# mika314/melonix

Measured on AMD Instinct MI355X. Metric: STFT+pitch+resynth frames/sec (48 kHz, 4096 FFT, 256 hop); % HBM roofline, higher is better.
Workload: dtype f32

## Files before the change

### melonix_amd/csrc/stft_core.h

```cpp
#pragma once
#include <stdint.h>
#include <type_traits>

#if defined(__HIPCC__)
#include <hip/hip_runtime.h>
#define MX_HD __host__ __device__ __forceinline__
namespace mx {
using cpx = float2;
}
#else
#define MX_HD inline __attribute__((always_inline))
namespace mx {
struct alignas(8) cpx {
  float x, y;
};
}
#endif

namespace mx {

#include "stft_consts.inc"

MX_HD cpx mk(float x, float y) {
  cpx r;
  r.x = x;
  r.y = y;
  return r;
}
MX_HD float fma_(float a, float b, float c) { return __builtin_fmaf(a, b, c); }
MX_HD cpx cadd(cpx a, cpx b) { return mk(a.x + b.x, a.y + b.y); }
MX_HD cpx csub(cpx a, cpx b) { return mk(a.x - b.x, a.y - b.y); }
MX_HD cpx cmul(cpx a, cpx b) { return mk(fma_(a.x, b.x, -(a.y * b.y)), fma_(a.x, b.y, a.y * b.x)); }
MX_HD float cnorm2(cpx a) { return fma_(a.x, a.x, a.y * a.y); }
MX_HD cpx cconj(cpx a) { return mk(a.x, -a.y); }
MX_HD cpx csel(bool c, cpx a, cpx b) { return mk(c ? a.x : b.x, c ? a.y : b.y); }
MX_HD float fast_sqrt(float x) {
#if defined(__HIP_DEVICE_COMPILE__)
  return __builtin_amdgcn_sqrtf(x);
#else
  return __builtin_sqrtf(x);
#endif
}
MX_HD constexpr int ilog2(int x) { return x <= 1 ? 0 : 1 + ilog2(x >> 1); }

}
#include "pk_math.h"
namespace mx {

template <int K>
MX_HD cpx mulw64(cpx a) {
  constexpr int k = ((K % 64) + 64) % 64;
  constexpr float h = 0.707106781187f;
  if constexpr (k == 0) return a;
  else if constexpr (k == 16) return mk(a.y, -a.x);
  else if constexpr (k == 32) return mk(-a.x, -a.y);
  else if constexpr (k == 48) return mk(-a.y, a.x);
  else if constexpr (k == 8) return mk(h * (a.x + a.y), h * (a.y - a.x));
  else if constexpr (k == 24) return mk(h * (a.y - a.x), -h * (a.x + a.y));
  else if constexpr (k == 40) return mk(-h * (a.x + a.y), h * (a.x - a.y));
  else if constexpr (k == 56) return mk(h * (a.x - a.y), h * (a.x + a.y));
  else {
    constexpr float c = kCos64[k], s = kSin64[k];
    return mk(fma_(a.x, c, a.y * s), fma_(a.y, c, -(a.x * s)));
  }
}

template <int K>
MX_HD void bfly_w64(cpx E, cpx O, cpx &out0, cpx &out1) {
  constexpr int k = ((K % 64) + 64) % 64;
  if constexpr (k == 0) {
    pk_bfly_1(E, O, out0, out1);
  } else if constexpr (k == 16) {
    pk_bfly_mi(E, O, out0, out1);
  } else if constexpr (k == 32) {
    pk_bfly_1(E, O, out1, out0);
  } else if constexpr (k == 48) {
    pk_bfly_mi(E, O, out1, out0);
  } else {
    pk_bfly_cs(E, O, mk(kCos64[k], kSin64[k]), out0, out1);
  }
}

template <int R, int Q>
struct Combine {
  static MX_HD void run(const cpx *E, const cpx *O, cpx *out) {
    bfly_w64<Q * 64 / R>(E[Q], O[Q], out[Q], out[Q + R / 2]);
    if constexpr (Q + 1 < R / 2) Combine<R, Q + 1>::run(E, O, out);
  }
};

template <int R>
struct Dft {
  static MX_HD void run(const cpx *in, cpx *out) {
    cpx e[R / 2], o[R / 2], E[R / 2], O[R / 2];
#pragma unroll
    for (int q = 0; q < R / 2; ++q) {
      e[q] = in[2 * q];
      o[q] = in[2 * q + 1];
    }
    Dft<R / 2>::run(e, E);
    Dft<R / 2>::run(o, O);
    Combine<R, 0>::run(E, O, out);
  }
};
template <>
struct Dft<2> {
  static MX_HD void run(const cpx *in, cpx *out) {
    pk_bfly_1(in[0], in[1], out[0], out[1]);
  }
};
template <>
struct Dft<1> {
  static MX_HD void run(const cpx *in, cpx *out) { out[0] = in[0]; }
};

template <int R, int S, int O0, bool CONJ>
struct DftTw {
  static MX_HD void run(const cpx *v, const cpx *w, cpx *out) {
    if constexpr (R == 2) {
      constexpr int i0 = O0, i1 = O0 + S;
      if constexpr (i0 == 0) pk_leaf0_tw<CONJ>(v[0], v[i1], w[i1], out[0], out[1]);
      else pk_leaf_tw<CONJ>(v[i0], w[i0], v[i1], w[i1], out[0], out[1]);
    } else {
      cpx E[R / 2], O[R / 2];
      DftTw<R / 2, 2 * S, O0, CONJ>::run(v, w, E);
      DftTw<R / 2, 2 * S, O0 + S, CONJ>::run(v, w, O);
      Combine<R, 0>::run(E, O, out);
    }
  }
};

template <int N_, int E_>
struct Plan {
  static constexpr int N = N_;
  static constexpr int M = N / 2;
  static constexpr int E = E_;
  static constexpr int T = M / E;
  static constexpr int R3 = E / 2;
  static constexpr int R1 = (N == 4096) ? 16 : 32;
  static constexpr int R2 = M / (R1 * R3);
  static constexpr int NS3 = R1 * R2;
  static constexpr int NB1 = E / R1;
  static constexpr int NB2 = E / R2;
  static constexpr int TW2 = (R2 - 1) * R1;
  static constexpr int TW3 = (R3 - 1) * NS3;
  static constexpr int L1 = ilog2(R1);
  static_assert(N == 4096 || N == 16384 || N == 32768, "supported FFT sizes");
  static_assert((N == 4096) ? E == 16 : E == 32, "supported points per thread");
  static_assert(R1 * R2 * R3 == M && R2 <= E && R1 <= E && T % 64 == 0, "radix plan must cover M");
};

template <class P>
MX_HD constexpr bool t1_padded() { return P::R1 == 32; }
template <class P>
MX_HD constexpr int t1_size() { return t1_padded<P>() ? P::M + P::M / 32 : P::M; }
template <class P>
MX_HD int t1_index(int i) {
  if constexpr (t1_padded<P>()) return i + (i >> 5);
  else return i ^ ((i >> P::L1) & 15);
}

struct alignas(4) f2u {
  float x, y;
};
template <bool ALIGNED8>
MX_HD cpx ld_pair(const float *base, int i) {
  const char *a = reinterpret_cast<const char *>(base) + (size_t)(4u * (unsigned)i);
  if constexpr (ALIGNED8) {
    return *reinterpret_cast<const cpx *>(a);
  } else {
    const f2u u = *reinterpret_cast<const f2u *>(a);
    return mk(u.x, u.y);
  }
}

MX_HD float ld_one(const float *base, int i) {
  return *reinterpret_cast<const float *>(reinterpret_cast<const char *>(base) + (size_t)(4u * (unsigned)i));
}

template <class P, int WSTEP, bool ALIGNED8>
MX_HD void load_frame(int t, cpx (&Y)[P::E], const float *x, const float *w) {
#pragma unroll
  for (int e = 0; e < P::E; ++e) {
    const int p = 2 * (t + P::T * e);
    cpx xs, ws;
    if constexpr (ALIGNED8 && WSTEP == 1) {
      xs = ld_pair<true>(x, p);
      ws = ld_pair<true>(w, p);
    } else {
      xs = ld_pair<false>(x, p);
      if constexpr (WSTEP == 1) {
        ws = ld_pair<false>(w, p);
      } else {
        const f2u wu = *reinterpret_cast<const f2u *>(w - p - 1);
        ws = mk(wu.y, wu.x);
      }
    }
    Y[e] = pk_mul(xs, ws);
  }
}

template <int T>
MX_HD constexpr float win_grow(int e) {
  return T == 64 ? kWinGrow64[e] : T == 128 ? kWinGrow128[e] : T == 256 ? kWinGrow256[e] : kWinGrow512[e];
}
template <class P, bool CLAMP = true>
MX_HD cpx geo_weight(cpx a0, int e) {
  constexpr float sc = 0.5f / (float)P::N;
  const float g = e == 0 ? 1.0f : win_grow<P::T>(e);
  const cpx w = e == 0 ? a0 : mk(a0.x * g, a0.y * g);
  if constexpr (!CLAMP) {
    return w;
  } else {
    const unsigned sb = __builtin_bit_cast(unsigned, sc), xb = __builtin_bit_cast(unsigned, w.x), yb = __builtin_bit_cast(unsigned, w.y);
    return mk(__builtin_bit_cast(float, xb < sb ? xb : sb), __builtin_bit_cast(float, yb < sb ? yb : sb));
  }
}
template <class P>
MX_HD int geo_clamped_slots(int hop) { return (hop + 2 * P::T - 1) / (2 * P::T); }
constexpr int kGeoTail = 2;
template <class P, bool ALIGNED8>
MX_HD void load_frame_geo(int t, cpx (&Y)[P::E], const float *x, const float *wb, int hop) {
  static_assert(P::T == 64 || P::T == 128 || P::T == 256 || P::T == 512, "growth table per T");
  static_assert(P::E <= 32, "growth table length");
  const cpx a0 = ld_pair<true>(wb, 2 * t);
  if (geo_clamped_slots<P>(hop) <= kGeoTail) {
#pragma unroll
    for (int e = 0; e < P::E; ++e) {
      const cpx xs = ld_pair<ALIGNED8>(x, 2 * (t + P::T * e));
      Y[e] = pk_mul(xs, e < P::E - kGeoTail ? geo_weight<P, false>(a0, e) : geo_weight<P, true>(a0, e));
    }
  } else {
#pragma unroll
    for (int e = 0; e < P::E; ++e) Y[e] = pk_mul(ld_pair<ALIGNED8>(x, 2 * (t + P::T * e)), geo_weight<P, true>(a0, e));
  }
}

template <class P>
MX_HD void apply_window_geo(int t, cpx (&Y)[P::E], const cpx (&xr)[P::E], const float *wb, int hop) {
  const cpx a0 = ld_pair<true>(wb, 2 * t);
  if (geo_clamped_slots<P>(hop) <= kGeoTail) {
#pragma unroll
    for (int e = 0; e < P::E; ++e)
      Y[e] = pk_mul(xr[e], e < P::E - kGeoTail ? geo_weight<P, false>(a0, e) : geo_weight<P, true>(a0, e));
  } else {
#pragma unroll
    for (int e = 0; e < P::E; ++e) Y[e] = pk_mul(xr[e], geo_weight<P, true>(a0, e));
  }
}

template <class P, bool ALIGNED8>
MX_HD void load_raw(int t, cpx (&xr)[P::E], const float *x) {
#pragma unroll
  for (int e = 0; e < P::E; ++e) {
    xr[e] = ld_pair<ALIGNED8>(x, 2 * (t + P::T * e));
  }
}
template <class P, int WSTEP, bool ALIGNED8>
MX_HD void apply_window(int t, cpx (&Y)[P::E], const cpx (&xr)[P::E], const float *w) {
#pragma unroll
  for (int e = 0; e < P::E; ++e) {
    const int p = 2 * (t + P::T * e);
    cpx ws;
    if constexpr (WSTEP == 1) {
      ws = ld_pair<ALIGNED8>(w, p);
    } else {
      const f2u wu = *reinterpret_cast<const f2u *>(w - p - 1);
      ws = mk(wu.y, wu.x);
    }
    Y[e] = pk_mul(xr[e], ws);
  }
}

template <class P>
MX_HD void pass1(const cpx (&Y)[P::E], cpx (&v)[P::E]) {
#pragma unroll
  for (int b = 0; b < P::NB1; ++b) {
    cpx in[P::R1], out[P::R1];
#pragma unroll
    for (int r = 0; r < P::R1; ++r) in[r] = Y[b + P::NB1 * r];
    Dft<P::R1>::run(in, out);
#pragma unroll
    for (int r = 0; r < P::R1; ++r) v[b * P::R1 + r] = out[r];
  }
}

template <class P, int HOP>
struct Slide {
  static constexpr int H = HOP / 2;
  static constexpr bool ok = (HOP > 0) && (HOP % 2 == 0) && (H % P::T == 0) && (2 * (H / P::T) <= P::E);
  static constexpr int D = ok ? H / P::T : 1;
};

template <class P, int HOP>
MX_HD void slide_edge(int t, const float *wtab, float inv_sc, cpx (&edge)[Slide<P, HOP>::D]) {
  using S = Slide<P, HOP>;
#pragma unroll
  for (int i = 0; i < S::D; ++i) {
    const int p = 2 * (t + P::T * (P::E - 2 * S::D + i));
    edge[i] = mk(wtab[p] * inv_sc, wtab[p + 1] * inv_sc);
  }
}

template <class P, int HOP>
MX_HD void slide_fetch(int t, const float *xe, cpx (&nx)[Slide<P, HOP>::D]) {
  using S = Slide<P, HOP>;
#pragma unroll
  for (int i = 0; i < S::D; ++i) nx[i] = *reinterpret_cast<const cpx *>(xe - HOP + 2 * (t + P::T * i));
}

template <class P, int HOP>
MX_HD void slide_step(cpx (&Y)[P::E], const cpx (&nx)[Slide<P, HOP>::D], const cpx (&edge)[Slide<P, HOP>::D],
                      float g, float sc) {
  using S = Slide<P, HOP>;
  const cpx gg = mk(g, g), ss = mk(sc, sc);
#pragma unroll
  for (int e = 0; e < P::E - 2 * S::D; ++e) Y[e] = pk_mul_xs(Y[e + S::D], gg);
#pragma unroll
  for (int i = 0; i < S::D; ++i) Y[P::E - 2 * S::D + i] = pk_mul(Y[P::E - S::D + i], edge[i]);
#pragma unroll
  for (int i = 0; i < S::D; ++i) Y[P::E - S::D + i] = pk_mul_xs(nx[i], ss);
}


template <class P>
struct Circ {
  static constexpr int W = 2 * P::T;
  static constexpr int CS = (P::T == 128) ? 4 : (P::T == 256) ? 3 : 2;
  static MX_HD bool ok(int hop) { return hop >= 1 && hop <= (CS - 1) * P::T && hop <= 2 * W; }
  static constexpr int slot(int k) { return (P::E - (CS - 1) + k) & (P::E - 1); }
};
template <class P>
struct CircGeo {
  int o;
  int s;
  int cr;
  int len;
};
template <class P>
MX_HD CircGeo<P> circ_geo(long long frame_end, int hop) {
  constexpr int W = Circ<P>::W;
  const long long start = frame_end - P::N;
  CircGeo<P> g;
  g.o = (int)(start & (long long)(W - 1));
  g.s = ((int)((start - hop) & (long long)(W - 1)) + hop) / W;
  g.len = 2 * hop;
  g.cr = (g.o - g.len) & (P::N - 1);
  return g;
}
template <class P>
MX_HD void circ_load_first(int t, cpx (&Y)[P::E], const float *xa, const float *w, int o) {
#pragma unroll
  for (int e = 0; e < P::E; ++e) {
    const int c2 = 2 * (t + P::T * e);
    const int q0 = (c2 - o) & (P::N - 1), q1 = (c2 + 1 - o) & (P::N - 1);
    Y[e] = mk(xa[q0] * w[q0], xa[q1] * w[q1]);
  }
}
template <class P>
MX_HD void circ_fetch(int t, const float *xs, const float *wt, const CircGeo<P> &g, float (&px)[2 * Circ<P>::CS],
                      float (&pw)[2 * Circ<P>::CS]) {
#pragma unroll
  for (int k = 0; k < Circ<P>::CS; ++k) {
    const int c2 = 2 * (t + P::T * Circ<P>::slot(k));
    int d0 = (c2 - g.cr) & (P::N - 1), d1 = (c2 + 1 - g.cr) & (P::N - 1);
    d0 = d0 < g.len ? d0 : g.len - 1;
    d1 = d1 < g.len ? d1 : g.len - 1;
    px[2 * k] = ld_one(xs, d0);
    px[2 * k + 1] = ld_one(xs, d1);
    pw[2 * k] = ld_one(wt, d0);
    pw[2 * k + 1] = ld_one(wt, d1);
  }
}
template <class P, int S>
MX_HD void circ_age(cpx (&Y)[P::E], cpx gg) {
  cpx head[S > 0 ? S : 1];
#pragma unroll
  for (int i = 0; i < S; ++i) head[i] = Y[i];
#pragma unroll
  for (int e = 0; e < P::E - S; ++e) Y[e] = pk_mul_xs(Y[e + S], gg);
#pragma unroll
  for (int i = 0; i < S; ++i) Y[P::E - S + i] = pk_mul_xs(head[i], gg);
}
template <class P>
MX_HD void circ_step(int t, cpx (&Y)[P::E], float decay, const CircGeo<P> &g, const float (&px)[2 * Circ<P>::CS],
                     const float (&pw)[2 * Circ<P>::CS]) {
  const cpx gg = mk(decay, decay);
  constexpr int SMAX = (Circ<P>::W - 1 + (Circ<P>::CS - 1) * P::T) / Circ<P>::W;
  static_assert(SMAX <= 2, "rotations by 0, 1 or 2 slots");
  if (g.s == 0) circ_age<P, 0>(Y, gg);
  else if (SMAX == 1 || g.s == 1) circ_age<P, 1>(Y, gg);
  else circ_age<P, 2>(Y, gg);
#pragma unroll
  for (int k = 0; k < Circ<P>::CS; ++k) {
    const int e = Circ<P>::slot(k);
    const int c2 = 2 * (t + P::T * e);
    const int d0 = (c2 - g.cr) & (P::N - 1), d1 = (c2 + 1 - g.cr) & (P::N - 1);
    const float n0 = px[2 * k] * pw[2 * k], n1 = px[2 * k + 1] * pw[2 * k + 1];
    Y[e] = mk(d0 < g.len ? n0 : Y[e].x, d1 < g.len ? n1 : Y[e].y);
  }
}


#if defined(__HIP_DEVICE_COMPILE__)
#define MX_LDS_ASM 1
typedef float mx_f2v __attribute__((ext_vector_type(2)));
template <int OFF>
__device__ __forceinline__ mx_f2v lds_rd64(uint32_t addr) {
  static_assert(OFF >= 0 && OFF < 163840, "LDS is 160 KiB");
  mx_f2v r;
  if constexpr (OFF < 65536) {
    asm volatile("ds_read_b64 %0, %1 offset:%2" : "=v"(r) : "v"(addr), "n"(OFF) : "memory");
  } else {
    const uint32_t hi = addr + (uint32_t)(OFF & ~65535);
    asm volatile("ds_read_b64 %0, %1 offset:%2" : "=v"(r) : "v"(hi), "n"(OFF & 65535) : "memory");
  }
  return r;
}
__device__ __forceinline__ uint32_t lds_addr(const void *p) {
  return (uint32_t)(uintptr_t)(const __attribute__((address_space(3))) void *)p;
}
template <int N>
__device__ __forceinline__ void lds_wait(mx_f2v (&q)[N]) {
  static_assert(N % 8 == 0, "tied in groups of 8");
  asm volatile("s_waitcnt lgkmcnt(0)" ::: "memory");
#pragma unroll
  for (int i = 0; i < N; i += 8)
    asm volatile("" : "+v"(q[i]), "+v"(q[i + 1]), "+v"(q[i + 2]), "+v"(q[i + 3]), "+v"(q[i + 4]),
                 "+v"(q[i + 5]), "+v"(q[i + 6]), "+v"(q[i + 7]));
}
#endif
template <int I, int N, class F>
MX_HD void static_for(F &&f) {
  if constexpr (I < N) {
    f(std::integral_constant<int, I>{});
    static_for<I + 1, N>(f);
  }
}

template <class P>
MX_HD void store_t1(int t, const cpx (&v)[P::E], cpx *lds) {
  if constexpr (t1_padded<P>()) {
    static_assert(P::R1 <= 32 && (P::T * P::R1) % 32 == 0, "T1 padding is one point per 32");
    cpx *const p = lds + (t * P::R1 + ((t * P::R1) >> 5));
#pragma unroll
    for (int b = 0; b < P::NB1; ++b) {
#pragma unroll
      for (int r = 0; r < P::R1; ++r) p[b * (P::T * P::R1 + P::T * P::R1 / 32) + r] = v[b * P::R1 + r];
    }
  } else {
    const unsigned B8 = (unsigned)((t * P::R1) ^ (t & 15)) << 3;
    char *const base = reinterpret_cast<char *>(lds);
#pragma unroll
    for (int r = 0; r < P::R1; ++r) {
      cpx *p = reinterpret_cast<cpx *>(base + (B8 ^ ((unsigned)r << 3)));
#pragma unroll
      for (int b = 0; b < P::NB1; ++b) p[b * P::T * P::R1] = v[b * P::R1 + r];
    }
  }
}

template <class P>
struct T1Read {
  static constexpr int S = P::M / P::R2;
  static constexpr int SP = t1_padded<P>() ? S + S / 32 : S;
  static constexpr int TP = t1_padded<P>() ? P::T + P::T / 32 : P::T;
  static constexpr int step = t1_padded<P>() ? 0 : ((S >> P::L1) & 15);
  static_assert(S % 32 == 0 && P::T % 32 == 0 && (step == 0 || step == 8), "T1 read is base(+alt base) + offset");
  static_assert(t1_padded<P>() || P::NB2 == 1, "the XOR layout's bases are written for one pass-2 butterfly per thread");
};

template <class P>
MX_HD void load_t1(int t, cpx (&v)[P::E], const cpx *lds) {
  using R = T1Read<P>;
  const int s1 = t1_index<P>(t);
#ifdef MX_LDS_ASM
  mx_f2v q[P::E];
  const uint32_t ae = lds_addr(lds + s1), ao = lds_addr(lds + (s1 ^ R::step));
  static_for<0, P::NB2>([&](auto bb) {
    constexpr int b = decltype(bb)::value;
    static_for<0, P::R2>([&](auto rr) {
      constexpr int r = decltype(rr)::value;
      q[b * P::R2 + r] = lds_rd64<(b * R::TP + r * R::SP) * 8>((r & 1) ? ao : ae);
    });
  });
  lds_wait(q);
#pragma unroll
  for (int i = 0; i < P::E; ++i) v[i] = mk(q[i].x, q[i].y);
#else
  const cpx *pe = lds + s1, *po = lds + (s1 ^ R::step);
#pragma unroll
  for (int b = 0; b < P::NB2; ++b) {
#pragma unroll
    for (int r = 0; r < P::R2; ++r) v[b * P::R2 + r] = ((r & 1) ? po : pe)[b * R::TP + r * R::SP];
  }
#endif
}

template <class P>
MX_HD void load_t1_tw2(int t, cpx (&v)[P::E], const cpx *lds, const cpx *ltw2, cpx (&w)[P::R2 - 1]) {
  static_assert(P::NB2 == 1 && P::E == P::R2 && P::E % 8 == 0, "one pass-2 butterfly per thread");
  using R = T1Read<P>;
  const int s1 = t1_index<P>(t);
#ifdef MX_LDS_ASM
  const uint32_t ae = lds_addr(lds + s1), ao = lds_addr(lds + (s1 ^ R::step));
  const uint32_t aw = lds_addr(ltw2 + (t & (P::R1 - 1)));
  mx_f2v q[2 * P::E];
  static_for<0, P::R2>([&](auto rr) {
    constexpr int r = decltype(rr)::value;
    q[r] = lds_rd64<r * R::SP * 8>((r & 1) ? ao : ae);
  });
  static_for<1, P::R2>([&](auto rr) {
    constexpr int r = decltype(rr)::value;
    q[P::E + r] = lds_rd64<(r - 1) * P::R1 * 8>(aw);
  });
  q[P::E] = mx_f2v{0.0f, 0.0f};
  lds_wait(q);
#pragma unroll
  for (int i = 0; i < P::E; ++i) v[i] = mk(q[i].x, q[i].y);
#pragma unroll
  for (int r = 1; r < P::R2; ++r) w[r - 1] = mk(q[P::E + r].x, q[P::E + r].y);
#else
  const cpx *pe = lds + s1, *po = lds + (s1 ^ R::step), *pw = ltw2 + (t & (P::R1 - 1));
#pragma unroll
  for (int r = 0; r < P::R2; ++r) v[r] = ((r & 1) ? po : pe)[r * R::SP];
#pragma unroll
  for (int r = 1; r < P::R2; ++r) w[r - 1] = pw[(r - 1) * P::R1];
#endif
}

template <class P>
MX_HD void pass2(int t, cpx (&v)[P::E], const cpx *tw2) {
#pragma unroll
  for (int b = 0; b < P::NB2; ++b) {
    const int j = t + P::T * b;
    const int k = j & (P::R1 - 1);
    cpx in[P::R2], w[P::R2], out[P::R2];
    w[0] = mk(1.0f, 0.0f);
#pragma unroll
    for (int r = 0; r < P::R2; ++r) in[r] = v[b * P::R2 + r];
#pragma unroll
    for (int r = 1; r < P::R2; ++r) {
      w[r] = tw2[(r - 1) * P::R1 + k];
    }
    DftTw<P::R2, 1, 0, false>::run(in, w, out);
#pragma unroll
    for (int r = 0; r < P::R2; ++r) v[b * P::R2 + r] = out[r];
  }
}

template <class P>
MX_HD void pass2_reg(cpx (&v)[P::E], const cpx (&w)[P::R2 - 1]) {
  static_assert(P::NB2 == 1, "one pass-2 butterfly per thread");
  cpx in[P::R2], ww[P::R2], out[P::R2];
  ww[0] = mk(1.0f, 0.0f);
#pragma unroll
  for (int r = 0; r < P::R2; ++r) in[r] = v[r];
#pragma unroll
  for (int r = 1; r < P::R2; ++r) ww[r] = w[r - 1];
  DftTw<P::R2, 1, 0, false>::run(in, ww, out);
#pragma unroll
  for (int r = 0; r < P::R2; ++r) v[r] = out[r];
}

template <class P>
MX_HD void store_t2(int t, const cpx (&v)[P::E], cpx *lds) {
#pragma unroll
  for (int b = 0; b < P::NB2; ++b) {
    const int j = t + P::T * b;
    const int k = j & (P::R1 - 1);
    const int base = (j - k) * P::R2 + k;
    cpx *p = lds + base;
#pragma unroll
    for (int r = 0; r < P::R2; ++r) p[r * P::R1] = v[b * P::R2 + r];
  }
}

template <class P>
MX_HD int k0p(int t) { return t; }
template <class P>
MX_HD int k0q(int t) { return t ? P::NS3 - t : P::NS3 / 2; }

template <class P>
MX_HD void load_t2(int t, cpx (&v)[P::E], const cpx *lds) {
  const int p = k0p<P>(t), q = k0q<P>(t);
#ifdef MX_LDS_ASM
  {
    const uint32_t pa = lds_addr(lds + p), qa = lds_addr(lds + q);
    mx_f2v w[P::E];
    static_for<0, P::R3>([&](auto rr) {
      constexpr int r = decltype(rr)::value;
      w[r] = lds_rd64<P::NS3 * r * 8>(pa);
      w[P::R3 + r] = lds_rd64<P::NS3 * r * 8>(qa);
    });
    lds_wait(w);
#pragma unroll
    for (int i = 0; i < P::E; ++i) v[i] = mk(w[i].x, w[i].y);
  }
#else
  const cpx *pp = lds + p, *qq = lds + q;
#pragma unroll
  for (int r = 0; r < P::R3; ++r) {
    v[r] = pp[P::NS3 * r];
    v[P::R3 + r] = qq[P::NS3 * r];
  }
#endif
}

template <class P>
MX_HD constexpr int q_index(int r) { return P::R3 + ((r + 1) & (P::R3 - 1)); }

template <class P>
MX_HD void fetch_tw3(int t, const cpx *tw3, cpx (&w)[P::R3 - 1]) {
  const int col = t ? t : P::NS3 / 2;
#pragma unroll
  for (int r = 1; r < P::R3; ++r) w[r - 1] = tw3[(r - 1) * P::NS3 + col];
}
template <class P>
MX_HD void fetch_tw3_bases(int t, const cpx *tw3, cpx (&wb)[6]) {
  static_assert(P::R3 == 16, "two-level pass-3 twiddles are written for radix 16");
  const int col = t ? t : P::NS3 / 2;
  constexpr int rr[6] = {1, 2, 3, 4, 8, 12};
#pragma unroll
  for (int i = 0; i < 6; ++i) wb[i] = tw3[(rr[i] - 1) * P::NS3 + col];
}
template <class P, bool MAY0>
MX_HD void pass3_reg(int t, cpx (&v)[P::E], const cpx (&w)[P::R3 - 1]);
template <class P, bool MAY0 = true>
MX_HD void pass3_bases(int t, cpx (&v)[P::E], const cpx (&wb)[6]) {
  cpx w[P::R3 - 1];
#pragma unroll
  for (int r = 1; r < P::R3; ++r) {
    const int hi = r >> 2, lo = r & 3;
    if (hi == 0) w[r - 1] = wb[lo - 1];
    else if (lo == 0) w[r - 1] = wb[2 + hi];
    else w[r - 1] = pk_cmul2(wb[2 + hi], wb[lo - 1]);
  }
  pass3_reg<P, MAY0>(t, v, w);
}
template <class P, bool MAY0 = true>
MX_HD void pass3_reg(int t, cpx (&v)[P::E], const cpx (&w)[P::R3 - 1]) {
  constexpr int R = P::R3;
  const bool t0 = MAY0 && (t == 0);
  cpx inp[R], inq[R], wp[R], wq[R], out[R];
  wp[0] = wq[0] = mk(1.0f, 0.0f);
#pragma unroll
  for (int r = 0; r < R; ++r) {
    inp[r] = v[r];
    inq[r] = v[R + r];
  }
#pragma unroll
  for (int r = 1; r < R; ++r) {
    wp[r] = csel(t0, mk(1.0f, 0.0f), w[r - 1]);
    wq[r] = w[r - 1];
  }
  DftTw<R, 1, 0, false>::run(inp, wp, out);
#pragma unroll
  for (int r = 0; r < R; ++r) v[r] = out[r];
  DftTw<R, 1, 0, true>::run(inq, wq, out);
#pragma unroll
  for (int r = 0; r < R; ++r) v[R + r] = out[r];
}

template <class P, int S>
struct PostSlot {
  static MX_HD void run(bool t0, const cpx (&v)[P::E], const cpx (&u)[P::R3], float (&mg)[P::E]) {
    constexpr int R = P::R3, H = R / 2;
    cpx A, B;
    if constexpr (S < H) {
      A = csel(t0, v[q_index<P>(S)], v[S]);
      B = v[q_index<P>(R - 1 - S)];
    } else {
      A = csel(t0, v[S - H], v[S]);
      B = csel(t0, v[(3 * H - S) & (R - 1)], v[q_index<P>(R - 1 - S)]);
    }
    const cpx n2 = pk_split_norm2(A, B, u[S]);
    mg[2 * S] = fast_sqrt(n2.x);
    mg[2 * S + 1] = fast_sqrt(n2.y);
    if constexpr (S == H) {
      const cpx z = v[H];
      const float m = fast_sqrt(cnorm2(z)) * 2.0f;
      mg[2 * S + 1] = t0 ? m : mg[2 * S + 1];
    }
    if constexpr (S + 1 < R) PostSlot<P, S + 1>::run(t0, v, u, mg);
  }
};

template <class P, bool MAY0 = true>
MX_HD void post(int t, const cpx (&v)[P::E], const cpx (&u)[P::R3], float (&mg)[P::E]) {
  PostSlot<P, 0>::run(MAY0 && t == 0, v, u, mg);
}

template <class P, int S>
struct PostFly {
  static MX_HD void run(cpx lo, cpx hi, cpx (&u)[P::R3]) {
    constexpr int k = ((32 / P::R3) * S) % 64;
    const cpx b = S < P::R3 / 2 ? lo : hi;
    if constexpr (k == 0) u[S] = b;
    else if constexpr (k == 16) u[S] = mk(b.y, -b.x);
    else u[S] = pk_rot_cs(b, mk(kCos64[k], kSin64[k]));
    if constexpr (S + 1 < P::R3) PostFly<P, S + 1>::run(lo, hi, u);
  }
};
template <class P>
MX_HD void post_bases(int t, const cpx *ubase, cpx &lo, cpx &hi) {
  if (t) {
    lo = ubase[t];
    hi = lo;
  } else {
    constexpr int k = 16 / P::R3;
    lo = mk(kSin64[k], kCos64[k]);
    hi = mk(-1.0f, 0.0f);
  }
}
template <class P, bool MAY0 = true>
MX_HD void post_fly(int t, const cpx (&v)[P::E], cpx lo, cpx hi, float (&mg)[P::E]) {
  cpx u[P::R3];
  PostFly<P, 0>::run(lo, MAY0 ? hi : lo, u);
  PostSlot<P, 0>::run(MAY0 && t == 0, v, u, mg);
}

template <class P, int S>
struct PostSlotC {
  static MX_HD void run(bool t0, const cpx (&v)[P::E], const cpx (&u)[P::R3], cpx (&X)[P::E]) {
    constexpr int R = P::R3, H = R / 2;
    cpx A, B;
    if constexpr (S < H) {
      A = csel(t0, v[q_index<P>(S)], v[S]);
      B = v[q_index<P>(R - 1 - S)];
    } else {
      A = csel(t0, v[S - H], v[S]);
      B = csel(t0, v[(3 * H - S) & (R - 1)], v[q_index<P>(R - 1 - S)]);
    }
    const cpx Sm = pk_add_cj(A, B);
    const cpx Dm = pk_sub_cj(A, B);
    const cpx D = pk_cmul<false>(Dm, u[S]);
    X[2 * S] = pk_sub(Sm, D);
    X[2 * S + 1] = cconj(pk_add(Sm, D));
    if constexpr (S == H) {
      const cpx z = v[H];
      X[2 * S + 1] = csel(t0, mk(2.0f * z.x, -2.0f * z.y), X[2 * S + 1]);
    }
    if constexpr (S + 1 < R) PostSlotC<P, S + 1>::run(t0, v, u, X);
  }
};
template <class P, bool MAY0 = true>
MX_HD void post_cplx(int t, const cpx (&v)[P::E], const cpx (&u)[P::R3], cpx (&X)[P::E]) {
  PostSlotC<P, 0>::run(MAY0 && t == 0, v, u, X);
}

template <class P>
MX_HD void out_bases(int t, int &lo, int &hi) {
  lo = t ? t : P::NS3 / 2;
  hi = t ? t : -(P::R3 / 2) * P::NS3;
}
template <class P>
MX_HD int out_bin(int t, int o) {
  int lo, hi;
  out_bases<P>(t, lo, hi);
  const int s = o >> 1;
  int k = (s < P::R3 / 2 ? lo : hi) + P::NS3 * s;
  if (o & 1) {
    k = P::M - k;
    if (k == P::M) k = P::M / 2;
  }
  return k;
}
template <class P>
MX_HD uint32_t band_mask(int t, int kmin, int kmax) {
  uint32_t m = 0;
#pragma unroll
  for (int o = 0; o < P::E; ++o) {
    const int k = out_bin<P>(t, o);
    m |= (k >= kmin && k <= kmax) ? (1u << o) : 0u;
  }
  return m;
}
MX_HD unsigned long long pick_key(float mag, int bin, int kmin, int kmax) {
  const unsigned in = (bin >= kmin && bin <= kmax) ? 0xffffffffu : 0u;
  return ((unsigned long long)(__builtin_bit_cast(unsigned, mag) & in) << 32) | ((0x7fffffffu - (unsigned)bin) & in);
}
MX_HD unsigned long long row_pick_key(int b0, float m0, float m1, float m2, float m3, int kmin, int kmax) {
  unsigned long long best = pick_key(m0, b0, kmin, kmax);
  const unsigned long long k1 = pick_key(m1, b0 + 1, kmin, kmax), k2 = pick_key(m2, b0 + 2, kmin, kmax),
                           k3 = pick_key(m3, b0 + 3, kmin, kmax);
  best = k1 > best ? k1 : best;
  best = k2 > best ? k2 : best;
  best = k3 > best ? k3 : best;
  return best;
}

template <class P, int S>
struct PostTw {
  static MX_HD void run(cpx lo, cpx hi, cpx (&u)[P::R3]) {
    u[S] = mulw64<(32 / P::R3) * S>(S < P::R3 / 2 ? lo : hi);
    if constexpr (S + 1 < P::R3) PostTw<P, S + 1>::run(lo, hi, u);
  }
};
template <class P>
MX_HD void post_twiddles(int t, const cpx *ubase, cpx (&u)[P::R3]) {
  cpx lo, hi;
  if (t) {
    lo = ubase[t];
    hi = lo;
  } else {
    constexpr int k = 16 / P::R3;
    lo = mk(kSin64[k], kCos64[k]);
    hi = mk(-1.0f, 0.0f);
  }
  PostTw<P, 0>::run(lo, hi, u);
}

}
```

### melonix_amd/csrc/stft_kernel_impl.h

```cpp
#pragma once
#include <hip/hip_runtime.h>

#include "colormap_core.h"
#include "kernels.h"
#include "stft_core.h"
#include "stft_tables.h"

#define MX_BARRIER() __syncthreads()

namespace mx {

template <bool MAXOP>
__device__ __forceinline__ unsigned wave_reduce_u32(unsigned k) {
  constexpr unsigned ident = MAXOP ? 0u : 0xffffffffu;
#define MX_DPP_STEP(CTRL, ROWS)                                                                      \
  {                                                                                                  \
    const unsigned o = (unsigned)__builtin_amdgcn_update_dpp((int)ident, (int)k, CTRL, ROWS, 0xf, false); \
    k = MAXOP ? (o > k ? o : k) : (o < k ? o : k);                                                   \
  }
  MX_DPP_STEP(0xB1, 0xf)
  MX_DPP_STEP(0x4E, 0xf)
  MX_DPP_STEP(0x141, 0xf)
  MX_DPP_STEP(0x140, 0xf)
  MX_DPP_STEP(0x142, 0xa)
  MX_DPP_STEP(0x143, 0xc)
#undef MX_DPP_STEP
  return (unsigned)__builtin_amdgcn_readlane((int)k, 63);
}
__device__ __forceinline__ unsigned long long wave_max_u64(unsigned long long k) {
  const unsigned hi = (unsigned)(k >> 32), lo = (unsigned)k;
  const unsigned mhi = wave_reduce_u32<true>(hi);
  const unsigned long long tie = __ballot(hi == mhi);
  unsigned mlo;
  if (__builtin_popcountll(tie) == 1) mlo = (unsigned)__builtin_amdgcn_readlane((int)lo, __builtin_ctzll(tie));
  else mlo = wave_reduce_u32<true>(hi == mhi ? lo : 0u);
  return ((unsigned long long)mhi << 32) | mlo;
}

template <int IMM, bool NT = true>
__device__ __forceinline__ void st_row_nt(const float *base, unsigned off, float x) {
  static_assert(IMM >= -4096 && IMM <= 4095, "global_store immediate offset");
#if defined(__HIP_DEVICE_COMPILE__)
  if constexpr (NT) asm volatile("global_store_dword %0, %1, %2 offset:%3 nt" : : "v"(off), "v"(x), "s"(base), "n"(IMM) : "memory");
  else asm volatile("global_store_dword %0, %1, %2 offset:%3" : : "v"(off), "v"(x), "s"(base), "n"(IMM) : "memory");
#endif
}

template <class P, int MODE, int HOP, int WPE, bool DEFER = false, bool PREFETCH = false, bool CMAP = false, bool DIRECT = false,
          bool CIRC = false, bool ROWPICK = false>
__global__ __launch_bounds__(P::T) __attribute__((amdgpu_waves_per_eu(WPE, WPE)))
void stft_kernel(const StftArgs a0) {
  const StftArgs &a = a0;
  using C = P;
  constexpr int N = P::N;
  constexpr int NW = C::T / 64;
  constexpr int kRed = (NW > 1) ? ((NW + 1) / 2) * 2 : 0;
  constexpr bool kTw3Bases = (P::R3 == 16);
  constexpr int kTw2 = ((C::TW2 + 1) / 2) * 2;
  static_assert(P::R3 == 16 || P::R3 == 8, "twiddle placement per plan");
  static_assert(!DIRECT || (NW > 1 && !DEFER && !CMAP), "direct row stores: multi-wave, non-deferred plans");
  static_assert(!ROWPICK || (DEFER && NW > 1 && !CMAP && !DIRECT && C::M / 4 / C::T >= 1 && C::T >= 128),
                "row-side pitch pick: the deferred two-wave plan, rows without texels");
  static_assert(!CIRC || (MODE != kRanges && HOP == 0 && !PREFETCH && !CMAP), "circular window: bulk modes");
  constexpr int IMG = t1_size<C>();
  __shared__ __attribute__((aligned(16))) float2 lds[IMG + kRed + (DEFER ? C::M / 2 : 0) + kTw2];
  float *const lout = reinterpret_cast<float *>(DEFER ? lds + IMG + kRed : lds);
  float2 *const ltw2 = lds + IMG + kRed + (DEFER ? C::M / 2 : 0);

  const int t_ = threadIdx.x;
  const bool wave0 = __builtin_amdgcn_readfirstlane(t_) < 64;
  cpx u[kTw3Bases ? 1 : P::R3];
  cpx ulo;
  cpx w3r[kTw3Bases ? 1 : P::R3 - 1], w3base[6];
  if constexpr (kTw3Bases) {
    cpx uhi_unused;
    post_bases<P>(t_, a.ubase, ulo, uhi_unused);
    fetch_tw3_bases<P>(t_, a.tw3, w3base);
  } else {
    post_twiddles<P>(t_, a.ubase, *reinterpret_cast<cpx(*)[P::R3]>(&u));
    fetch_tw3<P>(t_, a.tw3, *reinterpret_cast<cpx(*)[P::R3 - 1]>(&w3r));
  }
  uint32_t bmask_ = 0;
  uint32_t umask = 0;
  if constexpr (!ROWPICK) {
    bmask_ = band_mask<P>(t_, a.kmin, a.kmax);
#pragma unroll
    for (int o = 0; o < P::E; ++o) umask |= (__ballot((bmask_ >> o) & 1u) != 0ull) ? (1u << o) : 0u;
    umask = __builtin_amdgcn_readfirstlane(umask);
  }
  constexpr bool kSlide = (MODE == kBulkAligned) && (HOP > 0) && Slide<P, (HOP > 0 ? HOP : 2)>::ok;
  constexpr int SD = Slide<P, (HOP > 0 ? HOP : 2)>::D;
  constexpr float kSc = 0.5f / (float)N;
  for (int i = t_; i < C::TW2; i += C::T) ltw2[i] = a.tw2[i];
  MX_BARRIER();

  unsigned lb = blockIdx.x;
  {
    const unsigned nb = gridDim.x, xcd = lb & 7u, q = nb >> 3, r = nb & 7u;
    lb = (xcd < r ? xcd * (q + 1) : r * (q + 1) + (xcd - r) * q) + (lb >> 3);
  }
  const int64_t f0 = (int64_t)lb * a.frames_per_block;
  const int64_t f1 = (f0 + a.frames_per_block < a.count) ? f0 + a.frames_per_block : a.count;

  cpx Y[P::E];
  cpx edge[SD], nx[SD];
  if constexpr (kSlide) {
    const int64_t e0 = (a.first_frame + f0 + 1) * (int64_t)HOP;
    if (f0 < f1) load_frame<P, 1, true>(t_, Y, a.audio + MX_AUDIO_PAD + (e0 - N), a.wtab);
    slide_edge<P, HOP>(t_, a.wtab, 2.0f * (float)N, edge);
  }

  unsigned long long *const red = reinterpret_cast<unsigned long long *>(lds + IMG);
  auto flush_pitch = [&](int64_t fr, int tt) {
    if (!ROWPICK && a.pitch && tt == 0) {
      unsigned long long b = red[0];
#pragma unroll
      for (int i = 1; i < NW; ++i) b = red[i] > b ? red[i] : b;
      mx_pitch p;
      p.bin = 0x7fffffff - (int)(unsigned)(b & 0xffffffffull);
      p.mag = __uint_as_float((unsigned)(b >> 32));
      a.pitch[fr] = p;
    }
  };
  const bool want_rows = a.mags != nullptr || (CMAP && a.rgb != nullptr);
  auto flush_row = [&](int64_t fr, int tt) {
    if (want_rows) {
      using f32x4 = float __attribute__((ext_vector_type(4)));
      const f32x4 *l4 = reinterpret_cast<const f32x4 *>(lout) + tt;
      f32x4 *row4 = reinterpret_cast<f32x4 *>(a.mags + (size_t)fr * (size_t)(N / 2)) + tt;
      f32x4 q[C::M / 4 / C::T];
#pragma unroll
      for (int i = 0; i < C::M / 4 / C::T; ++i) q[i] = l4[C::T * i];
      if (!CMAP || a.mags) {
#pragma unroll
        for (int i = 0; i < C::M / 4 / C::T; ++i) {
          __builtin_nontemporal_store(q[i], &row4[C::T * i]);
        }
      }
      if constexpr (ROWPICK) {
        if (wave0) {
          const unsigned long long b = wave_max_u64(row_pick_key(4 * tt, q[0].x, q[0].y, q[0].z, q[0].w, a.kmin, a.kmax));
          if (tt == 0) {
            mx_pitch p;
            p.bin = 0x7fffffff - (int)(unsigned)(b & 0xffffffffull);
            p.mag = __uint_as_float((unsigned)(b >> 32));
            a.pitch[fr] = p;
          }
        }
      }
      if constexpr (CMAP) {
        if (a.rgb) {
          uint32_t *trow = reinterpret_cast<uint32_t *>(a.rgb + (size_t)fr * (size_t)(N / 2) * 3) + 3 * tt;
#pragma unroll 1
          for (int i = 0; i < C::M / 4 / C::T; ++i) {
            uint32_t w3[3];
            texel4(q[i].x, q[i].y, q[i].z, q[i].w, a.cmap_k, w3);
            uint32_t *o = trow + 3 * C::T * i;
            o[0] = w3[0];
            o[1] = w3[1];
            o[2] = w3[2];
          }
        }
      }
    }
  };

  auto frame_ptrs = [&](int64_t fr, int zo, const float *&x, const float *&w) {
    if constexpr (MODE == kRanges) {
      const int s = a.ranges[2 * fr], e = a.ranges[2 * fr + 1];
      const bool outside = (e <= 0) || ((int64_t)e - N >= a.n);
      x = outside ? a.audio : a.audio + MX_AUDIO_PAD + ((int64_t)e - N);
      int64_t d0 = (int64_t)N - ((int64_t)e - (int64_t)s);
      d0 = d0 < (int64_t)(N - 1 - kWOff) ? (int64_t)(N - 1 - kWOff) : d0;
      d0 = d0 > (int64_t)(kWDmax + kWTail) ? (int64_t)(kWDmax + kWTail) : d0;
      w = a.wext + kWOff + d0;
    } else {
      const int64_t e = (a.first_frame + fr + 1) * (int64_t)a.hop;
      x = a.audio + MX_AUDIO_PAD + (e - N);
      w = a.wtab + zo;
    }
  };
  float cpx_[2 * Circ<P>::CS], cpw_[2 * Circ<P>::CS];
  if constexpr (CIRC) {
    if (f0 < f1) {
      const int64_t pe = (a.first_frame + f0 + 1) * (int64_t)a.hop;
      circ_load_first<P>(t_, Y, a.audio + MX_AUDIO_PAD + (pe - N), a.wtab, circ_geo<P>(pe, a.hop).o);
    }
  }
  cpx xr[(PREFETCH && !kSlide) ? P::E : 1];
  if constexpr (PREFETCH && !kSlide) {
    if (f0 < f1) {
      const float *x0;
      const float *w0;
      frame_ptrs(f0, 0, x0, w0);
      load_raw<P, (MODE == kBulkAligned)>(t_, xr, x0);
    }
  }

  for (int64_t f = f0; f < f1; ++f) {
    int t = t_;
    unsigned bmask = bmask_;
    int zoff = 0;
    asm volatile("" : "+v"(t), "+v"(bmask), "+s"(zoff));
    int out_lo, out_hi;
    out_bases<P>(t, out_lo, out_hi);

    if constexpr (CIRC) {
      if (f > f0) {
        const int64_t pe = (a.first_frame + f + 1) * (int64_t)a.hop;
        const CircGeo<P> geo = circ_geo<P>(pe, a.hop);
        circ_fetch<P>(t, a.audio + MX_AUDIO_PAD + (pe - 2 * (int64_t)a.hop), a.wtab + zoff + (N - 2 * a.hop), geo, cpx_, cpw_);
        circ_step<P>(t, Y, a.decay, geo, cpx_, cpw_);
      }
    } else if constexpr (kSlide) {
      if (f > f0) slide_step<P, HOP>(Y, nx, edge, a.decay, kSc);
      if (f + 1 < f1) slide_fetch<P, HOP>(t, a.audio + MX_AUDIO_PAD + (a.first_frame + f + 2) * (int64_t)HOP, nx);
    } else {
      const float *x;
      const float *w;
      frame_ptrs(f, zoff, x, w);
      if constexpr (PREFETCH) {
        if constexpr (MODE == kRanges) apply_window<P, -1, false>(t, Y, xr, w);
        else apply_window_geo<P>(t, Y, xr, a.wtab + N + zoff, a.hop);
      } else if constexpr (MODE == kRanges) {
        load_frame<P, -1, false>(t, Y, x, w);
      } else {
        load_frame_geo<P, (MODE == kBulkAligned)>(t, Y, x, a.wtab + N + zoff, a.hop);
      }
    }

    cpx v[P::E];
    pass1<P>(Y, v);
    constexpr bool kTw2Batch = (P::NB2 == 1);
    store_t1<P>(t, v, lds);
    MX_BARRIER();
    if constexpr (DEFER || DIRECT) {
      if (f > f0) flush_pitch(f - 1, t);
    }
    if constexpr (kTw2Batch) {
      cpx w2[P::R2 - 1];
      load_t1_tw2<P>(t, v, lds, ltw2, w2);
      if constexpr (DEFER) {
        if (f > f0) flush_row(f - 1, t);
      }
      MX_BARRIER();
      pass2_reg<P>(v, w2);
    } else {
      load_t1<P>(t, v, lds);
      if constexpr (DEFER) {
        if (f > f0) flush_row(f - 1, t);
      }
      MX_BARRIER();
      pass2<P>(t, v, ltw2);
    }
    store_t2<P>(t, v, lds);
    MX_BARRIER();
    load_t2<P>(t, v, lds);
    MX_BARRIER();
    float mg[P::E];
    if (NW == 1 || wave0) {
      if constexpr (kTw3Bases) {
        pass3_bases<P, true>(t, v, w3base);
        post_fly<P, true>(t, v, ulo, csel(t == 0, mk(-1.0f, 0.0f), ulo), mg);
      } else {
        pass3_reg<P, true>(t, v, *reinterpret_cast<cpx(*)[P::R3 - 1]>(&w3r));
        post<P, true>(t, v, *reinterpret_cast<cpx(*)[P::R3]>(&u), mg);
      }
    } else {
      if constexpr (kTw3Bases) {
        pass3_bases<P, false>(t, v, w3base);
        post_fly<P, false>(t, v, ulo, ulo, mg);
      } else {
        pass3_reg<P, false>(t, v, *reinterpret_cast<cpx(*)[P::R3 - 1]>(&w3r));
        post<P, false>(t, v, *reinterpret_cast<cpx(*)[P::R3]>(&u), mg);
      }
    }

    if constexpr (PREFETCH && !kSlide) {
      if (f + 1 < f1) {
        const float *xn;
        const float *wn;
        frame_ptrs(f + 1, zoff, xn, wn);
        load_raw<P, (MODE == kBulkAligned)>(t, xr, xn);
      }
    }

    unsigned long long best = 0ull;
    if (!ROWPICK && a.pitch) {
      const unsigned klo = 0x7fffffffu - (unsigned)out_lo, khi = 0x7fffffffu - (unsigned)out_hi;
      const unsigned nlo = 0x7fffffffu - (unsigned)(C::M - out_lo), nhi = 0x7fffffffu - (unsigned)(C::M - out_hi);
#pragma unroll
      for (int s = 0; s < C::R3; ++s) {
        constexpr int H = C::R3 / 2;
        if (!((umask >> (2 * s)) & 3u)) continue;
        const unsigned b0 = (s < H ? klo : khi) - (unsigned)(C::NS3 * s);
        unsigned b1 = (s < H ? nlo : nhi) + (unsigned)(C::NS3 * s);
        if (s == H) b1 = (t == 0) ? 0x7fffffffu - (unsigned)(C::M / 2) : b1;
        const unsigned v0 = (unsigned)((int)(bmask << (31 - 2 * s)) >> 31);
        const unsigned v1 = (unsigned)((int)(bmask << (31 - (2 * s + 1))) >> 31);
        const unsigned long long k0 = ((unsigned long long)(__float_as_uint(mg[2 * s]) & v0) << 32) | (b0 & v0);
        const unsigned long long k1 = ((unsigned long long)(__float_as_uint(mg[2 * s + 1]) & v1) << 32) | (b1 & v1);
        best = k0 > best ? k0 : best;
        best = k1 > best ? k1 : best;
      }
      best = wave_max_u64(best);
      if constexpr (NW > 1) {
        if ((t & 63) == 0) red[t >> 6] = best;
      }
    }

    if constexpr (DIRECT) {
      if (want_rows) {
        const float *row = a.mags + (size_t)f * (size_t)(N / 2);
        constexpr int H = C::R3 / 2;
        constexpr int STEP = 4 * C::NS3;
        constexpr int G = 8192 / STEP;
        static_assert((STEP == 4096 || STEP == 2048) && H % G == 0, "slot groups share an offset through the store's immediate");
        const unsigned blo = 4u * (unsigned)out_lo, bhi = 4u * (unsigned)(out_hi + C::NS3 * H);
        const unsigned nlo = 4u * (unsigned)(C::M - out_lo), nhi = 4u * (unsigned)(C::M - out_hi - C::NS3 * H);
        static_for<0, C::R3>([&](auto ss) {
          constexpr int s = decltype(ss)::value;
          constexpr int sl = s < H ? s : s - H;
          constexpr int su = (sl & ~(G - 1)) + G / 2, sd = (sl & ~(G - 1)) + G / 2 - 1;
          const unsigned o0 = (s < H ? blo : bhi) + (unsigned)(su * STEP);
          unsigned o1 = (s < H ? nlo : nhi) - (unsigned)(sd * STEP);
          if constexpr (s == H) {
            o1 = (t == 0) ? (unsigned)(4 * (C::M / 2)) + (unsigned)((sl - sd) * STEP) : o1;
          }
          st_row_nt<(sl - su) * STEP>(row, o0, mg[2 * s]);
          st_row_nt<-(sl - sd) * STEP, false>(row, o1, mg[2 * s + 1]);
        });
      }
    } else if (want_rows) {
      float *plo = lout + out_lo, *phi = lout + out_hi;
      float *mlo = lout + (C::M - out_lo), *mhi = lout + (C::M - out_hi);
#pragma unroll
      for (int s = 0; s < C::R3; ++s) {
        constexpr int H = C::R3 / 2;
        (s < H ? plo : phi)[C::NS3 * s] = mg[2 * s];
        if (s == H) (t == 0 ? lout + C::M / 2 : mhi - C::NS3 * H)[0] = mg[2 * s + 1];
        else (s < H ? mlo : mhi)[-C::NS3 * s] = mg[2 * s + 1];
      }
    }
    if constexpr (!DEFER && !DIRECT) {
      if (want_rows) {
        MX_BARRIER();
        flush_row(f, t);
        MX_BARRIER();
      } else {
        MX_BARRIER();
      }
      if constexpr (NW > 1) {
        flush_pitch(f, t);
      } else if (a.pitch && t == 0) {
        mx_pitch p;
        p.bin = 0x7fffffff - (int)(unsigned)(best & 0xffffffffull);
        p.mag = __uint_as_float((unsigned)(best >> 32));
        a.pitch[f] = p;
      }
    }
  }
  if constexpr (DEFER || DIRECT) {
    if (f0 < f1) {
      MX_BARRIER();
      flush_pitch(f1 - 1, t_);
      if constexpr (DEFER) flush_row(f1 - 1, t_);
    }
  }
}


}
```

Measured before the change: 336.7 million.

## Hoist pass-3 twiddle selects, precompute band masks, scalar-address row stores, reorder LDS

Moves the per-frame t==0 twiddle selection in pass 3 out of the frame loop into precomputed registers. Replaces per-frame kmin/kmax band tests in the row-side pitch pick with wave ballots computed once and expanded via inverse_ballot. Row flushes now use a scalar base address plus immediate offsets, and the LDS layout for the deferred row buffer and reduction slots is swapped. Magnitude LDS stores are regrouped so that the t==0 special case runs outside the loop. The hoisting adds live registers, which could affect occupancy.

After: 343.7 million (median of 6 runs). 1.02x the previous value.

```diff
diff --git a/melonix_amd/csrc/stft_core.h b/melonix_amd/csrc/stft_core.h
--- a/melonix_amd/csrc/stft_core.h
+++ b/melonix_amd/csrc/stft_core.h
@@ -638,8 +638,15 @@
   }
   pass3_reg<P, MAY0>(t, v, w);
 }
-template <class P, bool MAY0 = true>
-MX_HD void pass3_reg(int t, cpx (&v)[P::E], const cpx (&w)[P::R3 - 1]) {
+template <class P, int KH>
+MX_HD void pass3_wp0(int t, const cpx (&w)[P::R3 - 1], cpx (&wph)[KH > 0 ? KH : 1]) {
+  static_assert(KH >= 0 && KH <= P::R3 - 1, "at most every twiddle");
+  wph[0] = mk(1.0f, 0.0f);
+#pragma unroll
+  for (int r = 1; r <= KH; ++r) wph[r - 1] = csel(t == 0, mk(1.0f, 0.0f), w[r - 1]);
+}
+template <class P, bool MAY0 = true, int KH = 0>
+MX_HD void pass3_reg(int t, cpx (&v)[P::E], const cpx (&w)[P::R3 - 1], const cpx (&wph)[KH > 0 ? KH : 1]) {
   constexpr int R = P::R3;
   const bool t0 = MAY0 && (t == 0);
   cpx inp[R], inq[R], wp[R], wq[R], out[R];
@@ -651,7 +658,7 @@
   }
 #pragma unroll
   for (int r = 1; r < R; ++r) {
-    wp[r] = csel(t0, mk(1.0f, 0.0f), w[r - 1]);
+    wp[r] = (MAY0 && r <= KH) ? wph[r <= KH ? r - 1 : 0] : csel(t0, mk(1.0f, 0.0f), w[r - 1]);
     wq[r] = w[r - 1];
   }
   DftTw<R, 1, 0, false>::run(inp, wp, out);
@@ -660,6 +667,11 @@
   DftTw<R, 1, 0, true>::run(inq, wq, out);
 #pragma unroll
   for (int r = 0; r < R; ++r) v[R + r] = out[r];
+}
+template <class P, bool MAY0>
+MX_HD void pass3_reg(int t, cpx (&v)[P::E], const cpx (&w)[P::R3 - 1]) {
+  const cpx none[1] = {mk(1.0f, 0.0f)};
+  pass3_reg<P, MAY0, 0>(t, v, w, none);
 }
 
 template <class P, int S>
@@ -776,9 +788,12 @@
   }
   return m;
 }
+MX_HD unsigned long long pick_key(float mag, int bin, bool in_band) {
+  const unsigned in = in_band ? 0xffffffffu : 0u;
+  return ((unsigned long long)(__builtin_bit_cast(unsigned, mag) & in) << 32) | ((0x7fffffffu - (unsigned)bin) & in);
+}
 MX_HD unsigned long long pick_key(float mag, int bin, int kmin, int kmax) {
-  const unsigned in = (bin >= kmin && bin <= kmax) ? 0xffffffffu : 0u;
-  return ((unsigned long long)(__builtin_bit_cast(unsigned, mag) & in) << 32) | ((0x7fffffffu - (unsigned)bin) & in);
+  return pick_key(mag, bin, bin >= kmin && bin <= kmax);
 }
 MX_HD unsigned long long row_pick_key(int b0, float m0, float m1, float m2, float m3, int kmin, int kmax) {
   unsigned long long best = pick_key(m0, b0, kmin, kmax);
@@ -788,6 +803,23 @@
   best = k2 > best ? k2 : best;
   best = k3 > best ? k3 : best;
   return best;
+}
+MX_HD unsigned long long row_pick_key(int b0, float m0, float m1, float m2, float m3, bool in0, bool in1, bool in2, bool in3) {
+  unsigned long long best = pick_key(m0, b0, in0);
+  const unsigned long long k1 = pick_key(m1, b0 + 1, in1), k2 = pick_key(m2, b0 + 2, in2), k3 = pick_key(m3, b0 + 3, in3);
+  best = k1 > best ? k1 : best;
+  best = k2 > best ? k2 : best;
+  best = k3 > best ? k3 : best;
+  return best;
+}
+MX_HD unsigned row_band_mask(int b0, int kmin, int kmax) {
+  unsigned m = 0;
+#pragma unroll
+  for (int j = 0; j < 4; ++j) m |= (b0 + j >= kmin && b0 + j <= kmax) ? (1u << j) : 0u;
+  return m;
+}
+MX_HD unsigned long long row_pick_key(int b0, float m0, float m1, float m2, float m3, unsigned mask) {
+  return row_pick_key(b0, m0, m1, m2, m3, (mask & 1u) != 0, (mask & 2u) != 0, (mask & 4u) != 0, (mask & 8u) != 0);
 }
 
 template <class P, int S>
diff --git a/melonix_amd/csrc/stft_kernel_impl.h b/melonix_amd/csrc/stft_kernel_impl.h
--- a/melonix_amd/csrc/stft_kernel_impl.h
+++ b/melonix_amd/csrc/stft_kernel_impl.h
@@ -64,10 +64,12 @@
   static_assert(!CIRC || (MODE != kRanges && HOP == 0 && !PREFETCH && !CMAP), "circular window: bulk modes");
   constexpr int IMG = t1_size<C>();
   __shared__ __attribute__((aligned(16))) float2 lds[IMG + kRed + (DEFER ? C::M / 2 : 0) + kTw2];
-  float *const lout = reinterpret_cast<float *>(DEFER ? lds + IMG + kRed : lds);
+  float *const lout = reinterpret_cast<float *>(DEFER ? lds + IMG : lds);
   float2 *const ltw2 = lds + IMG + kRed + (DEFER ? C::M / 2 : 0);
 
   const int t_ = threadIdx.x;
+  constexpr bool kSlide = (MODE == kBulkAligned) && (HOP > 0) && Slide<P, (HOP > 0 ? HOP : 2)>::ok;
+  constexpr int SD = Slide<P, (HOP > 0 ? HOP : 2)>::D;
   const bool wave0 = __builtin_amdgcn_readfirstlane(t_) < 64;
   cpx u[kTw3Bases ? 1 : P::R3];
   cpx ulo;
@@ -80,6 +82,9 @@
     post_twiddles<P>(t_, a.ubase, *reinterpret_cast<cpx(*)[P::R3]>(&u));
     fetch_tw3<P>(t_, a.tw3, *reinterpret_cast<cpx(*)[P::R3 - 1]>(&w3r));
   }
+  constexpr int kTw3Hoist = (!kTw3Bases && ROWPICK) ? ((kSlide && SD > 1) ? 3 : P::R3 - 1) : 0;
+  cpx w3p[kTw3Hoist > 0 ? kTw3Hoist : 1];
+  if constexpr (!kTw3Bases) pass3_wp0<P, kTw3Hoist>(t_, *reinterpret_cast<cpx(*)[P::R3 - 1]>(&w3r), w3p);
   uint32_t bmask_ = 0;
   uint32_t umask = 0;
   if constexpr (!ROWPICK) {
@@ -88,8 +93,12 @@
     for (int o = 0; o < P::E; ++o) umask |= (__ballot((bmask_ >> o) & 1u) != 0ull) ? (1u << o) : 0u;
     umask = __builtin_amdgcn_readfirstlane(umask);
   }
-  constexpr bool kSlide = (MODE == kBulkAligned) && (HOP > 0) && Slide<P, (HOP > 0 ? HOP : 2)>::ok;
-  constexpr int SD = Slide<P, (HOP > 0 ? HOP : 2)>::D;
+  unsigned long long rin[4] = {0ull, 0ull, 0ull, 0ull};
+  if constexpr (ROWPICK) {
+    const unsigned rm = row_band_mask(4 * t_, a.kmin, a.kmax);
+#pragma unroll
+    for (int j = 0; j < 4; ++j) rin[j] = __ballot((rm >> j) & 1u);
+  }
   constexpr float kSc = 0.5f / (float)N;
   for (int i = t_; i < C::TW2; i += C::T) ltw2[i] = a.tw2[i];
   MX_BARRIER();
@@ -110,7 +119,7 @@
     slide_edge<P, HOP>(t_, a.wtab, 2.0f * (float)N, edge);
   }
 
-  unsigned long long *const red = reinterpret_cast<unsigned long long *>(lds + IMG);
+  unsigned long long *const red = reinterpret_cast<unsigned long long *>(lds + IMG + (DEFER ? C::M / 2 : 0));
   auto flush_pitch = [&](int64_t fr, int tt) {
     if (!ROWPICK && a.pitch && tt == 0) {
       unsigned long long b = red[0];
@@ -123,6 +132,7 @@
     }
   };
   const bool want_rows = a.mags != nullptr || (CMAP && a.rgb != nullptr);
+  constexpr bool kRowSaddr = (C::M / 4 / C::T == 4) && (C::T * 16 == 2048);
   auto flush_row = [&](int64_t fr, int tt) {
     if (want_rows) {
       using f32x4 = float __attribute__((ext_vector_type(4)));
@@ -132,14 +142,33 @@
 #pragma unroll
       for (int i = 0; i < C::M / 4 / C::T; ++i) q[i] = l4[C::T * i];
       if (!CMAP || a.mags) {
-#pragma unroll
-        for (int i = 0; i < C::M / 4 / C::T; ++i) {
-          __builtin_nontemporal_store(q[i], &row4[C::T * i]);
+        if constexpr (kRowSaddr) {
+          uintptr_t mid = reinterpret_cast<uintptr_t>(a.mags + (size_t)fr * (size_t)(N / 2)) + 4096;
+#if defined(__HIP_DEVICE_COMPILE__)
+          asm volatile("" : "+s"(mid));
+          using gchar = __attribute__((address_space(1))) char;
+          using gf32x4 = __attribute__((address_space(1))) f32x4;
+#else
+          using gchar = char;
+          using gf32x4 = f32x4;
+#endif
+          const unsigned off = 16u * (unsigned)tt;
+#pragma unroll
+          for (int i = 0; i < 4; ++i)
+            __builtin_nontemporal_store(q[i], reinterpret_cast<gf32x4 *>(reinterpret_cast<gchar *>(mid) + off + (2048 * i - 4096)));
+        } else {
+#pragma unroll
+          for (int i = 0; i < C::M / 4 / C::T; ++i) {
+            __builtin_nontemporal_store(q[i], &row4[C::T * i]);
+          }
         }
       }
       if constexpr (ROWPICK) {
         if (wave0) {
-          const unsigned long long b = wave_max_u64(row_pick_key(4 * tt, q[0].x, q[0].y, q[0].z, q[0].w, a.kmin, a.kmax));
+          const unsigned long long b = wave_max_u64(row_pick_key(
+              4 * tt, q[0].x, q[0].y, q[0].z, q[0].w, __builtin_amdgcn_inverse_ballot_w64(rin[0]),
+              __builtin_amdgcn_inverse_ballot_w64(rin[1]), __builtin_amdgcn_inverse_ballot_w64(rin[2]),
+              __builtin_amdgcn_inverse_ballot_w64(rin[3])));
           if (tt == 0) {
             mx_pitch p;
             p.bin = 0x7fffffff - (int)(unsigned)(b & 0xffffffffull);
@@ -263,7 +292,7 @@
         pass3_bases<P, true>(t, v, w3base);
         post_fly<P, true>(t, v, ulo, csel(t == 0, mk(-1.0f, 0.0f), ulo), mg);
       } else {
-        pass3_reg<P, true>(t, v, *reinterpret_cast<cpx(*)[P::R3 - 1]>(&w3r));
+        pass3_reg<P, true, kTw3Hoist>(t, v, *reinterpret_cast<cpx(*)[P::R3 - 1]>(&w3r), w3p);
         post<P, true>(t, v, *reinterpret_cast<cpx(*)[P::R3]>(&u), mg);
       }
     } else {
@@ -334,13 +363,13 @@
     } else if (want_rows) {
       float *plo = lout + out_lo, *phi = lout + out_hi;
       float *mlo = lout + (C::M - out_lo), *mhi = lout + (C::M - out_hi);
-#pragma unroll
-      for (int s = 0; s < C::R3; ++s) {
-        constexpr int H = C::R3 / 2;
-        (s < H ? plo : phi)[C::NS3 * s] = mg[2 * s];
-        if (s == H) (t == 0 ? lout + C::M / 2 : mhi - C::NS3 * H)[0] = mg[2 * s + 1];
-        else (s < H ? mlo : mhi)[-C::NS3 * s] = mg[2 * s + 1];
-      }
+      constexpr int H = C::R3 / 2;
+#pragma unroll
+      for (int s = 0; s < C::R3; ++s) (s < H ? plo : phi)[C::NS3 * s] = mg[2 * s];
+#pragma unroll
+      for (int s = 0; s < C::R3; ++s)
+        if (s != H) (s < H ? mlo : mhi)[-C::NS3 * s] = mg[2 * s + 1];
+      (t == 0 ? lout + C::M / 2 : mhi - C::NS3 * H)[0] = mg[2 * H + 1];
     }
     if constexpr (!DEFER && !DIRECT) {
       if (want_rows) {
```
